# TensorSpeech/TensorFlowASR

Measured on AMD Instinct MI355X. Metric: audio-hours/sec (train step) Conformer-M RNN-T, higher is better.
Workload: dtype bf16; 1 GPU; Conformer-M transducer full train step (fwd+RNN-T loss+bwd+Adam), LibriSpeech-shaped 16 kHz utterances, 32/GPU, padding=batch, SpecAugment on, dropout 0.1; global_batch=32, parallelism=dp1, params=32461288

## Files before the change

### include/tfasr_hip.h

```cpp
#ifndef TFASR_HIP_H_
#define TFASR_HIP_H_

#include <stddef.h>
#include <stdint.h>

#ifdef __cplusplus
extern "C" {
#endif

#define TFASR_ABI_VERSION 44

typedef enum {
  TFASR_STATUS_SUCCESS = 0,
  TFASR_STATUS_INVALID_VALUE = 1,
  TFASR_STATUS_EXECUTION_FAILED = 2,
  TFASR_STATUS_UNSUPPORTED = 3
} tfasr_status_t;

typedef enum { TFASR_F32 = 0, TFASR_BF16 = 1 } tfasr_dtype_t;

const char* tfasr_status_string(int status);
int tfasr_abi_version(void);
size_t tfasr_launch_count(void);

// ... 3 lines not shown
                    int blank, int dtype, float* costs, void* workspace, size_t workspace_bytes,
                    void* stream);
int tfasr_rnnt_loss_packed_coef(const int32_t* labels, const int32_t* label_len, const int32_t* logit_len, const float* grad_scale,
                                const long* cell_off, long total_cells, const float* lse_part, int lse_parts, const float* pick, int B, int T,
                                int U1, int V, int blank, float* costs, float* coef, void* workspace, size_t workspace_bytes, void* stream);
int tfasr_rnnt_row_labels(const int32_t* labels, const int32_t* label_len, const int32_t* logit_len, const long* cell_off,
                          long total_cells, int B, int T, int U1, int V, int32_t* row_label, void* stream);
int tfasr_rnnt_loss_packed_stats(const void* logits, void* grads, const int32_t* labels, const int32_t* label_len,
                                 const int32_t* logit_len, const float* grad_scale, const long* cell_off, long total_cells,
                                 const float* lse_part, int lse_parts, const float* pick, int B, int T, int U1, int V, int blank,
                                 int dtype, float* costs, void* workspace, size_t workspace_bytes, void* stream);
int tfasr_rnnt_loss_packed(const void* logits, void* grads, const int32_t* labels, const int32_t* label_len,
                           const int32_t* logit_len, const float* grad_scale, const long* cell_off, long total_cells, int B,
                           int T, int U1, int V, int blank, int dtype, float* costs, void* workspace,
                           size_t workspace_bytes, void* stream);

int tfasr_ctc_loss_workspace_size(int B, int T, int U, int V, size_t* bytes);
int tfasr_ctc_loss(const void* logits, void* grads, const int32_t* labels, const int32_t* label_len,
                   const int32_t* logit_len, const float* grad_scale, int B, int T, int U, int V, int blank, int dtype,
                   float* costs, void* workspace, size_t workspace_bytes, void* stream);
int tfasr_ctc_greedy_decode(const void* logits, const int32_t* logit_len, int32_t* workspace_argmax, int32_t* tokens,
                            int32_t* tokens_len, int B, int T, int V, int blank, int dtype, void* stream);
int tfasr_ctc_greedy_decode_detail(const void* logits, const int32_t* logit_len, int32_t* workspace, int32_t* tokens, int32_t* tokens_len,
                                   int32_t* starts, int32_t* ends, float* tok_logp, float* tok_entropy, float* score, int B, int T, int V,
                                   int blank, int dtype, void* stream);

typedef enum { TFASR_ACT_NONE = 0, TFASR_ACT_SWISH = 1, TFASR_ACT_TANH = 2, TFASR_ACT_SIGMOID = 3, TFASR_ACT_TANH_OUT = 4,
               TFASR_ACT_FACTOR = 5  } tfasr_act_t;

typedef struct {
// ... 487 lines not shown
```

### tensorflowasr_amd/csrc/align.hip

```cpp
#include "common.h"
#include "lattice_lp.h"
#include <algorithm>

namespace {

typedef unsigned long long u64;

inline size_t align256(size_t x) { return (x + 255) & ~(size_t)255; }

constexpr int kRnntMaxU1 = TFASR_ALIGN_MAX_U1;
constexpr int kCtcMaxU = TFASR_ALIGN_CTC_MAX_U;

inline int rnnt_wave_e(int U1) { return U1 <= 64 ? 1 : (U1 <= 128 ? 2 : (U1 <= 256 ? 4 : 0)); }
inline int rnnt_dec_nw(int U1) { const int e = rnnt_wave_e(U1); return e ? e : (U1 + 63) / 64; }
inline size_t rnnt_dec_bytes(int B, int T, int U1) { return align256((size_t)B * ((size_t)T + U1) * rnnt_dec_nw(U1) * sizeof(u64)); }
inline int ctc_dec_nw(int U) { return (2 * U + 1 + 63) / 64; }

template <int E>
__global__ __launch_bounds__(64) void rnnt_viterbi_wave_kernel(const float* __restrict__ blank_lp, const float* __restrict__ truth_lp,
                                                               const int32_t* __restrict__ label_len, const int32_t* __restrict__ logit_len,
                                                               const long* __restrict__ cell_off, int Tm, int U1m, u64* __restrict__ dec,
                                                               long dec_stride, float* __restrict__ score) {
  const int b = blockIdx.x, lane = threadIdx.x;
  const int Tl = min(logit_len[b], Tm), Ul = max(min(label_len[b], U1m - 1), 0);
// ... 263 lines not shown
  if (!labels || !label_len || !logit_len || !score || !workspace || (U1 > 1 && (!frames || !label_lp))) return TFASR_STATUS_INVALID_VALUE;
  if (V <= 1 || blank < 0 || blank >= V) return TFASR_STATUS_INVALID_VALUE;
  const int st = rnnt_shape_status(B, T, U1);
  if (st != TFASR_STATUS_SUCCESS) return st;
  if (blank != 0) return TFASR_STATUS_UNSUPPORTED;
  const long nrows = cell_off ? total_cells : (long)B * T * U1;
  if (nrows <= 0 || nrows > (long)B * T * U1) return TFASR_STATUS_INVALID_VALUE;
  const size_t seg = align256((size_t)nrows * sizeof(float));
  if (workspace_bytes < 3 * seg + rnnt_dec_bytes(B, T, U1)) return TFASR_STATUS_INVALID_VALUE;
  hipStream_t stream = (hipStream_t)stream_;
  char* ws = (char*)workspace;
  float* lse = (float*)ws;
  float* bl = (float*)(ws + seg);
  float* tr = (float*)(ws + 2 * seg);
  const int lp = tfasr_detail::rnnt_lattice_logprobs(logits, labels, label_len, logit_len, cell_off, nrows, B, T, U1, V, dtype, lse_part, lse_parts,
                                                     pick, lse, bl, tr, stream);
  if (lp != TFASR_STATUS_SUCCESS) return lp;
  return rnnt_walk(bl, tr, label_len, logit_len, cell_off, B, T, U1, frames, label_lp, score, (u64*)(ws + 3 * seg), stream);
}

}

extern "C" int tfasr_rnnt_align_workspace_size(int B, int T, int U1, int V, size_t* bytes) {
  if (!bytes || V <= 0) return TFASR_STATUS_INVALID_VALUE;
  const int st = rnnt_shape_status(B, T, U1);
  if (st != TFASR_STATUS_SUCCESS) return st;
  *bytes = 3 * align256((size_t)B * T * U1 * sizeof(float)) + rnnt_dec_bytes(B, T, U1);
  return TFASR_STATUS_SUCCESS;
}

extern "C" int tfasr_rnnt_align_lattice(const float* blank_lp, const float* truth_lp, const int32_t* label_len, const int32_t* logit_len,
// ... 72 lines not shown
```

### tensorflowasr_amd/csrc/elementwise.hip

```cpp
#include "common.h"
#include <stdlib.h>
#include <algorithm>

namespace {

inline int flat_grid(long n, int per = 256) { return (int)std::max<long>(1, std::min<long>((n + per - 1) / per, 256L * 16)); }

template <typename S, typename D>
__global__ __launch_bounds__(256) void cast_kernel(const S* __restrict__ src, D* __restrict__ dst, long n) {
  const long n8 = n / 8;
  for (long i = (long)blockIdx.x * blockDim.x + threadIdx.x; i < n8; i += (long)gridDim.x * blockDim.x) {
    float v[8];
    ld8(src + i * 8, v);
    st8(dst + i * 8, v);
  }
  for (long i = n8 * 8 + (long)blockIdx.x * blockDim.x + threadIdx.x; i < n; i += (long)gridDim.x * blockDim.x)
    Num<D>::st(dst + i, Num<S>::ld(src + i));
}

template <typename T>
__global__ __launch_bounds__(256) void dropout_kernel(const T* x, T* y, long n, float p, uint64_t seed) {
  const long n8 = n / 8;
  const float inv = 1.f / (1.f - p);
  for (long i = (long)blockIdx.x * blockDim.x + threadIdx.x; i < n8; i += (long)gridDim.x * blockDim.x) {
// ... 522 lines not shown
    const float r = sqrtf(-2.0f * __logf(u1));
    float sn, cs;
    __sincosf(6.283185307179586f * u2, &sn, &cs);
    x[i] += stddev * r * ((i & 1) ? sn : cs);
  }
}

__global__ __launch_bounds__(256) void sumsq_kernel(const float* __restrict__ p, long n, float* __restrict__ out) {
  __shared__ float red[16];
  float a = 0.f;
  for (long i = (long)blockIdx.x * blockDim.x + threadIdx.x; i < n; i += (long)gridDim.x * blockDim.x) a += p[i] * p[i];
  a = block_sum(a, red);
  if (threadIdx.x == 0) atomicAdd(out, a);
}

template <typename T>
__global__ __launch_bounds__(256) void specaug_kernel(T* __restrict__ x, const int32_t* __restrict__ fmask,
                                                      const int32_t* __restrict__ tmask, int nf, int nt, int B, int Tn,
                                                      int F, float mval) {
  const long n = (long)B * Tn * F;
  for (long i = (long)blockIdx.x * blockDim.x + threadIdx.x; i < n; i += (long)gridDim.x * blockDim.x) {
    const int f = (int)(i % F);
    const int t = (int)((i / F) % Tn);
    const int b = (int)(i / ((long)F * Tn));
    bool hit = false;
    for (int k = 0; k < nf; ++k) {
      const int f0 = fmask[(b * nf + k) * 2], fw = fmask[(b * nf + k) * 2 + 1];
      hit |= (f >= f0 && f < f0 + fw);
    }
    for (int k = 0; k < nt; ++k) {
      const int t0 = tmask[(b * nt + k) * 2], tw = tmask[(b * nt + k) * 2 + 1];
      hit |= (t >= t0 && t < t0 + tw);
    }
    if (hit) Num<T>::st(x + i, mval);
  }
}

}

#define DISPATCH_T(dtype, CALL_F32, CALL_BF16) \
  do { if ((dtype) == TFASR_F32) { CALL_F32; } else if ((dtype) == TFASR_BF16) { CALL_BF16; } else return TFASR_STATUS_INVALID_VALUE; } while (0)

extern "C" int tfasr_cast(const void* src, void* dst, long n, int src_dtype, int dst_dtype, void* stream_) {
  if (!src || !dst || n <= 0) return TFASR_STATUS_INVALID_VALUE;
  hipStream_t s = (hipStream_t)stream_;
  const int grid = flat_grid(n / 8 + 1);
  if (src_dtype == TFASR_F32 && dst_dtype == TFASR_BF16)
    TFASR_KLAUNCH((cast_kernel<float, bf16_t>), dim3(grid), dim3(256), 0, s, (const float*)src, (bf16_t*)dst, n);
  else if (src_dtype == TFASR_BF16 && dst_dtype == TFASR_F32)
// ... 313 lines not shown
  TFASR_CHECK_LAUNCH();
  return TFASR_STATUS_SUCCESS;
}

extern "C" int tfasr_sumsq(const float* p, long n, float* out, void* stream_) {
  if (!p || !out || n <= 0) return TFASR_STATUS_INVALID_VALUE;
  TFASR_KLAUNCH(sumsq_kernel, dim3(flat_grid(n)), dim3(256), 0, (hipStream_t)stream_, p, n, out);
  TFASR_CHECK_LAUNCH();
  return TFASR_STATUS_SUCCESS;
}

extern "C" int tfasr_specaugment(void* x, const int32_t* fmask, const int32_t* tmask, int nf, int nt, int B, int T,
                                 int F, float mask_value, int dtype, void* stream_) {
  if (!x || B <= 0 || T <= 0 || F <= 0 || (nf > 0 && !fmask) || (nt > 0 && !tmask)) return TFASR_STATUS_INVALID_VALUE;
  hipStream_t s = (hipStream_t)stream_;
  const int grid = flat_grid((long)B * T * F);
  DISPATCH_T(dtype,
             TFASR_KLAUNCH(specaug_kernel<float>, dim3(grid), dim3(256), 0, s, (float*)x, fmask, tmask, nf, nt, B, T, F, mask_value),
             TFASR_KLAUNCH(specaug_kernel<bf16_t>, dim3(grid), dim3(256), 0, s, (bf16_t*)x, fmask, tmask, nf, nt, B, T, F, mask_value));
  TFASR_CHECK_LAUNCH();
  return TFASR_STATUS_SUCCESS;
}

namespace {
template <typename T>
__global__ __launch_bounds__(256) void add_pe_kernel(const T* __restrict__ x, const float* __restrict__ pe, const int32_t* __restrict__ lengths,
                                                     T* __restrict__ y, int B, int Tn, int d) {
  const int d8 = d / 8;
  const long n8 = (long)B * Tn * d8;
  for (long i = (long)blockIdx.x * blockDim.x + threadIdx.x; i < n8; i += (long)gridDim.x * blockDim.x) {
    const int c = (int)(i % d8) * 8;
    const long row = i / d8;
    const int t = (int)(row % Tn), b = (int)(row / Tn);
    float v[8];
// ... 23 lines not shown
```

### tensorflowasr_amd/csrc/lattice_lp.h

```cpp
#pragma once
#include "common.h"

namespace tfasr_detail {

__attribute__((visibility("hidden"))) int rnnt_lattice_logprobs(const void* logits, const int32_t* labels, const int32_t* label_len,
                                                                const int32_t* logit_len, const long* cell_off, long nrows, int B, int T, int U1,
                                                                int V, int dtype, const float* lse_part, int lse_parts, const float* pick,
                                                                float* lse, float* blank_lp, float* truth_lp, hipStream_t stream);

__attribute__((visibility("hidden"))) int ctc_row_lse(const void* logits, float* lse, long rows, int V, int dtype, hipStream_t stream);

}
```

### tensorflowasr_amd/csrc/rnnt_loss.hip

```cpp
#include "common.h"
#include "lattice_lp.h"
#include <algorithm>
#include <stdlib.h>

namespace {

struct RowStat { float m, s; };

__device__ __forceinline__ void online_add(RowStat& st, float x) {
  if (x > st.m) { st.s = st.s * __expf(st.m - x) + 1.f; st.m = x; }
  else          { st.s += __expf(x - st.m); }
}
__device__ __forceinline__ void online_merge(RowStat& a, float m2, float s2) {
  const float m = fmaxf(a.m, m2);
  if (m == -INFINITY) { a.m = m; a.s = 0.f; return; }
  a.s = a.s * __expf(a.m - m) + s2 * __expf(m2 - m);
  a.m = m;
}

struct Cell { int b, t, u, Tl, Ul; bool valid; };
__device__ __forceinline__ Cell locate(long r, const long* __restrict__ cell_off, int B, int Tm, int U1,
                                       const int32_t* __restrict__ label_len, const int32_t* __restrict__ logit_len) {
  Cell c;
  if (cell_off) {
    int lo = 0, hi = B;
    while (hi - lo > 1) { const int mid = (lo + hi) >> 1; if (cell_off[mid] <= r) lo = mid; else hi = mid; }
    c.b = lo;
    c.Tl = min(logit_len[lo], Tm); c.Ul = min(label_len[lo], U1 - 1);
    const long q = r - cell_off[lo];
    c.t = (int)(q / (c.Ul + 1)); c.u = (int)(q % (c.Ul + 1));
    c.valid = true;
  } else {
    c.u = (int)(r % U1); c.t = (int)((r / U1) % Tm); c.b = (int)(r / ((long)U1 * Tm));
    c.Tl = min(logit_len[c.b], Tm); c.Ul = min(label_len[c.b], U1 - 1);
    c.valid = (c.t < c.Tl && c.u <= c.Ul);
  }
  return c;
}

template <typename T>
__global__ __launch_bounds__(256) void rnnt_logprobs_kernel(
    const T* __restrict__ logits, const int32_t* __restrict__ labels, const int32_t* __restrict__ label_len,
    const int32_t* __restrict__ logit_len, const long* __restrict__ cell_off, long nrows, int B, int Tm, int U1, int V,
    float* __restrict__ lse, float* __restrict__ blank_lp, float* __restrict__ truth_lp) {
  const int lane = threadIdx.x & 63;
  const long wave0 = (long)blockIdx.x * (blockDim.x >> 6) + (threadIdx.x >> 6);
  const long nwaves = (long)gridDim.x * (blockDim.x >> 6);
  const bool vec_ok = (V % 8 == 0);
  for (long r = wave0; r < nrows; r += nwaves) {
    const Cell cl = locate(r, cell_off, B, Tm, U1, label_len, logit_len);
    const int u = cl.u, b = cl.b;
    if (!cl.valid) continue;
    const T* row = logits + r * V;
    RowStat st{-INFINITY, 0.f};
    int lab = -1;
    if (u < U1 - 1) lab = min(max(labels[(long)b * (U1 - 1) + u], 0), V - 1);
    float x_blank = 0.f, x_truth = 0.f;
    bool from_regs = false;
    if (vec_ok && V <= 2 * 64 * 8) {
// ... 37 lines not shown
          ld8(row + v0, x);
#pragma unroll
          for (int i = 0; i < 8; ++i) online_add(st, x[i]);
        }
      } else {
        for (int v = lane; v < V; v += 64) online_add(st, Num<T>::ld(row + v));
      }
#pragma unroll
      for (int o = 32; o > 0; o >>= 1) {
        const float m2 = __shfl_xor(st.m, o, 64), s2 = __shfl_xor(st.s, o, 64);
        online_merge(st, m2, s2);
      }
    }
    if (lane == 0) {
      const float l = st.m + logf(st.s);
      lse[r] = l;
      blank_lp[r] = (from_regs ? x_blank : Num<T>::ld(row)) - l;
      float tr = -INFINITY;
      if (lab >= 0) tr = (from_regs ? x_truth : Num<T>::ld(row + lab)) - l;
      truth_lp[r] = tr;
    }
  }
}

__global__ __launch_bounds__(256) void rnnt_row_labels_kernel(const int32_t* __restrict__ labels, const int32_t* __restrict__ label_len,
                                                              const int32_t* __restrict__ logit_len, const long* __restrict__ cell_off,
                                                              long nrows, int B, int Tm, int U1, int V, int32_t* __restrict__ row_label) {
  for (long r = (long)blockIdx.x * blockDim.x + threadIdx.x; r < nrows; r += (long)gridDim.x * blockDim.x) {
    const Cell cl = locate(r, cell_off, B, Tm, U1, label_len, logit_len);
    int lab = -1;
    if (cl.valid && cl.u < cl.Ul) lab = min(max(labels[(long)cl.b * (U1 - 1) + cl.u], 0), V - 1);
    row_label[r] = lab;
  }
}

__global__ __launch_bounds__(256) void rnnt_stats_finalize_kernel(const float2* __restrict__ part, int nparts, const float* __restrict__ pick,
                                                                  const int32_t* __restrict__ label_len, const int32_t* __restrict__ logit_len,
                                                                  const long* __restrict__ cell_off, long nrows, int B, int Tm, int U1,
                                                                  float* __restrict__ lse, float* __restrict__ blank_lp, float* __restrict__ truth_lp) {
  if (nparts == 16) {
    const int li = threadIdx.x & 15;
    const long g0 = ((long)blockIdx.x * blockDim.x + threadIdx.x) >> 4, gs = ((long)gridDim.x * blockDim.x) >> 4;
    const long nr16 = (nrows + gs - 1) / gs * gs;
    for (long r = g0; r < nr16; r += gs) {
      const bool in = r < nrows;
      const float2 v = in ? part[r * 16 + li] : make_float2(-INFINITY, 0.f);
      const float mx = row16_max(v.x);
      const float sm = row16_sum(v.y > 0.f ? v.y * __expf(v.x - mx) : 0.f);
      if (in && li == 0) {
        const Cell cl = locate(r, cell_off, B, Tm, U1, label_len, logit_len);
        if (cl.valid) {
          const float l = mx + logf(sm);
          const float2 pk = *reinterpret_cast<const float2*>(pick + 2 * r);
          lse[r] = l;
          blank_lp[r] = pk.x - l;
          truth_lp[r] = (cl.u < cl.Ul) ? pk.y - l : -INFINITY;
        }
      }
    }
    return;
  }
  for (long r = (long)blockIdx.x * blockDim.x + threadIdx.x; r < nrows; r += (long)gridDim.x * blockDim.x) {
    const Cell cl = locate(r, cell_off, B, Tm, U1, label_len, logit_len);
    if (!cl.valid) continue;
    RowStat st{-INFINITY, 0.f};
    for (int c = 0; c < nparts; ++c) {
      const float2 v = part[r * nparts + c];
      online_merge(st, v.x, v.y);
    }
    const float l = st.m + logf(st.s);
    lse[r] = l;
    blank_lp[r] = pick[2 * r] - l;
    truth_lp[r] = (cl.u < cl.Ul) ? pick[2 * r + 1] - l : -INFINITY;
  }
}

__device__ __forceinline__ void lds_barrier() { asm volatile("s_waitcnt lgkmcnt(0)\n\ts_barrier" ::: "memory"); }

__global__ __launch_bounds__(1024) void rnnt_lattice_kernel(const float* __restrict__ blank_lp, const float* __restrict__ truth_lp,
                                    const int32_t* __restrict__ label_len, const int32_t* __restrict__ logit_len,
                                    const long* __restrict__ cell_off, int Tm, int U1m, float* __restrict__ alpha,
                                    float* __restrict__ beta, float* __restrict__ costs) {
  extern __shared__ float sh[];
  const int b = blockIdx.x;
  const int u = threadIdx.x;
  const int nthr = blockDim.x;
  const int Tl = min(logit_len[b], Tm), Ul = min(label_len[b], U1m - 1);
  const int U1 = cell_off ? Ul + 1 : U1m;
// ... 85 lines not shown
        lds_barrier();
      }
    }
  }
}

template <bool FAST>
__device__ __forceinline__ float lae_(float a, float b) {
  if constexpr (!FAST) return logaddexpf_(a, b);
  const float m = fmaxf(a, b);
  if (m == -INFINITY) return -INFINITY;
  const float e = __builtin_amdgcn_exp2f(-fabsf(a - b) * 1.44269504088896340736f);
  return m + __builtin_amdgcn_logf(1.0f + e) * 0.69314718055994530942f;
}

template <int E, bool FAST>
__global__ __launch_bounds__(64) void rnnt_lattice_wave_kernel(const float* __restrict__ blank_lp, const float* __restrict__ truth_lp,
                                                               const int32_t* __restrict__ label_len, const int32_t* __restrict__ logit_len,
                                                               const long* __restrict__ cell_off, int Tm, int U1m, float* __restrict__ alpha,
                                                               float* __restrict__ beta, float* __restrict__ costs) {
  const int b = blockIdx.x, lane = threadIdx.x;
  const int Tl = min(logit_len[b], Tm), Ul = min(label_len[b], U1m - 1);
  const int U1 = cell_off ? Ul + 1 : U1m;
  const long base = cell_off ? cell_off[b] : (long)b * Tm * U1m;
  const float* bl = blank_lp + base;
  const float* tr = truth_lp + base;
  if (Tl <= 0) { if (lane == 0 && blockIdx.y == 1) costs[b] = 0.f; return; }
  const int ndiag = Tl + Ul;
  constexpr int PF = E == 1 ? 32 : (E == 2 ? 16 : 8);
  float rb[PF][E], rt[PF][E];
  int ue[E], uc[E];
  bool ucol[E];
#pragma unroll
  for (int e = 0; e < E; ++e) { ue[e] = lane * E + e; uc[e] = min(ue[e], Ul); ucol[e] = ue[e] <= Ul; }
  float self[E];
#pragma unroll
  for (int e = 0; e < E; ++e) self[e] = -INFINITY;
  if (blockIdx.y == 0) {
    float* al = alpha + base;
    auto fetch = [&](int n, int e, float& fb, float& ft) {
      const int tc = min(max(n - ue[e], 0), Tl - 1);
      fb = bl[max(tc - 1, 0) * U1 + uc[e]];
      ft = tr[tc * U1 + max(uc[e] - 1, 0)];
    };
#pragma unroll
    for (int j = 0; j < PF; ++j)
#pragma unroll
      for (int e = 0; e < E; ++e) fetch(j, e, rb[j][e], rt[j][e]);
    for (int n0 = 0; n0 < ndiag; n0 += PF) {
#pragma unroll
      for (int j = 0; j < PF; ++j) {
        const int n = n0 + j;
        float left[E];
        left[0] = __int_as_float(__builtin_amdgcn_update_dpp(__float_as_int(-INFINITY), __float_as_int(self[E - 1]), 0x138 , 0xf, 0xf, false));
#pragma unroll
        for (int e = 1; e < E; ++e) left[e] = self[e - 1];
#pragma unroll
        for (int e = 0; e < E; ++e) {
          const int t = n - ue[e];
          const bool act = ucol[e] && t >= 0 && t < Tl;
          const float pb = rb[j][e], pt = rt[j][e];
          fetch(n + PF, e, rb[j][e], rt[j][e]);
          if (act) {
            float a;
            if (t == 0 && ue[e] == 0) a = 0.f;
            else {
              const float xb = (t > 0) ? self[e] + pb : -INFINITY;
              const float xt = (ue[e] > 0) ? left[e] + pt : -INFINITY;
              a = lae_<FAST>(xb, xt);
            }
            al[t * U1 + ue[e]] = a;
            self[e] = a;
          }
        }
      }
    }
  } else {
    float* be = beta + base;
    auto fetch = [&](int it, int e, float& fb, float& ft) {
      const int tc = min(max((ndiag - 1 - it) - ue[e], 0), Tl - 1);
      fb = bl[tc * U1 + uc[e]];
      ft = tr[tc * U1 + uc[e]];
    };
#pragma unroll
    for (int j = 0; j < PF; ++j)
#pragma unroll
      for (int e = 0; e < E; ++e) fetch(j, e, rb[j][e], rt[j][e]);
    for (int i0 = 0; i0 < ndiag; i0 += PF) {
#pragma unroll
      for (int j = 0; j < PF; ++j) {
        const int it = i0 + j;
        const int n = ndiag - 1 - it;
        float right[E];
        right[E - 1] = __int_as_float(__builtin_amdgcn_update_dpp(__float_as_int(-INFINITY), __float_as_int(self[0]), 0x130 , 0xf, 0xf, false));
#pragma unroll
        for (int e = 0; e + 1 < E; ++e) right[e] = self[e + 1];
#pragma unroll
        for (int e = 0; e < E; ++e) {
          const int t = n - ue[e];
          const bool act = ucol[e] && t >= 0 && t < Tl;
          const float pb = rb[j][e], pt = rt[j][e];
          fetch(it + PF, e, rb[j][e], rt[j][e]);
          if (act) {
            float v;
            if (t == Tl - 1 && ue[e] == Ul) v = pb;
            else {
              const float xb = (t + 1 < Tl) ? self[e] + pb : -INFINITY;
              const float xt = (ue[e] < Ul) ? right[e] + pt : -INFINITY;
              v = lae_<FAST>(xb, xt);
            }
            be[t * U1 + ue[e]] = v;
            self[e] = v;
            if (t == 0 && ue[e] == 0) costs[b] = -v;
          }
        }
      }
    }
  }
}

template <typename T>
__global__ __launch_bounds__(256) void rnnt_grad_kernel(
    const T* logits, T* grads, const int32_t* __restrict__ labels,
    const int32_t* __restrict__ label_len, const int32_t* __restrict__ logit_len,
    const float* __restrict__ grad_scale, const long* __restrict__ cell_off, long nrows, int B, int Tm, int U1, int V,
    const float* __restrict__ lse, const float* __restrict__ blank_lp, const float* __restrict__ truth_lp,
    const float* __restrict__ alpha, const float* __restrict__ beta) {
  const int lane = threadIdx.x & 63;
  const long wave0 = (long)blockIdx.x * (blockDim.x >> 6) + (threadIdx.x >> 6);
  const long nwaves = (long)gridDim.x * (blockDim.x >> 6);
  const bool vec_ok = (V % 8 == 0);
  for (long r = wave0; r < nrows; r += nwaves) {
    const Cell cl = locate(r, cell_off, B, Tm, U1, label_len, logit_len);
    const int u = cl.u, t = cl.t, b = cl.b, Tl = cl.Tl, Ul = cl.Ul;
    const int ustride = cell_off ? Ul + 1 : U1;
    const T* row = logits + r * V;
    T* out = grads + r * V;
    if (!cl.valid) {
      if (vec_ok) {
        const float z[8] = {0, 0, 0, 0, 0, 0, 0, 0};
        for (int v0 = lane * 8; v0 < V; v0 += 64 * 8) st8(out + v0, z);
      } else {
        for (int v = lane; v < V; v += 64) Num<T>::st(out + v, 0.f);
      }
      continue;
    }
    const long lb = cell_off ? cell_off[b] : (long)b * Tm * U1;
    const float b00 = beta[lb];
    const float a = alpha[r];
    float gb = 0.f, gt = 0.f;
    if (t < Tl - 1) gb = -__expf(a + beta[r + ustride] + blank_lp[r] - b00);
    else if (u == Ul) gb = -1.f;
    int lab = -1;
    if (u < Ul) {
      gt = -__expf(a + beta[r + 1] + truth_lp[r] - b00);
      lab = min(max(labels[(long)b * (U1 - 1) + u], 0), V - 1);
    }
    const float sc = grad_scale ? grad_scale[b] : 1.f;
    const float l = lse[r];
    const float ssum = gb + gt;
    if (vec_ok) {
      const float l2 = l * 1.4426950408889634f, k1 = -ssum * sc, gbs = gb * sc, gts = gt * sc;
      for (int v0 = lane * 8; v0 < V; v0 += 64 * 8) {
        float x[8];
        ld8(row + v0, x);
#pragma unroll
        for (int i = 0; i < 8; ++i) x[i] = __builtin_amdgcn_exp2f(x[i] * 1.4426950408889634f - l2) * k1;
        if (v0 == 0) x[0] += gbs;
        if (lab >= 0 && (lab >> 3) == (v0 >> 3)) {
          const int q = lab & 7;
// ... 5 lines not shown
    } else {
      for (int v = lane; v < V; v += 64) {
        float g = -__expf(Num<T>::ld(row + v) - l) * ssum;
        if (v == 0) g += gb;
        if (v == lab) g += gt;
        Num<T>::st(out + v, g * sc);
      }
    }
  }
}

__global__ __launch_bounds__(256) void rnnt_coef_kernel(
    const int32_t* __restrict__ label_len, const int32_t* __restrict__ logit_len, const float* __restrict__ grad_scale,
    const long* __restrict__ cell_off, long nrows, int B, int Tm, int U1, const float* __restrict__ lse, const float* __restrict__ blank_lp,
    const float* __restrict__ truth_lp, const float* __restrict__ alpha, const float* __restrict__ beta, float4* __restrict__ coef,
    const int32_t* __restrict__ labels = nullptr, int V = 0, int32_t* __restrict__ rlab = nullptr) {
  for (long r = (long)blockIdx.x * blockDim.x + threadIdx.x; r < nrows; r += (long)gridDim.x * blockDim.x) {
    const Cell cl = locate(r, cell_off, B, Tm, U1, label_len, logit_len);
    float4 c = make_float4(3.0e38f, 0.f, 0.f, 0.f);
    if (rlab) rlab[r] = (cl.valid && cl.u < cl.Ul) ? min(max(labels[(long)cl.b * (U1 - 1) + cl.u], 0), V - 1) : -1;
    if (cl.valid) {
      const int u = cl.u, t = cl.t, b = cl.b, Tl = cl.Tl, Ul = cl.Ul;
      const int ustride = cell_off ? Ul + 1 : U1;
      const long lb = cell_off ? cell_off[b] : (long)b * Tm * U1;
      const float b00 = beta[lb], a = alpha[r];
      float gb = 0.f, gt = 0.f;
      if (t < Tl - 1) gb = -__expf(a + beta[r + ustride] + blank_lp[r] - b00);
      else if (u == Ul) gb = -1.f;
      if (u < Ul) gt = -__expf(a + beta[r + 1] + truth_lp[r] - b00);
      const float sc = grad_scale ? grad_scale[b] : 1.f;
      c = make_float4(lse[r] * 1.4426950408889634f, -(gb + gt) * sc, gb * sc, gt * sc);
    }
    coef[r] = c;
  }
}

template <typename T>
__global__ __launch_bounds__(256) void rnnt_grad_apply_kernel(const T* __restrict__ logits, T* __restrict__ grads, const float4* __restrict__ coef,
                                                              const int32_t* __restrict__ rlab, long nrows, int V) {
  const int lane = threadIdx.x & 63;
  const long wave0 = (long)blockIdx.x * (blockDim.x >> 6) + (threadIdx.x >> 6);
  const long nwaves = (long)gridDim.x * (blockDim.x >> 6);
  constexpr int U = 2, MAXP = 2;
  for (long r0 = wave0; r0 < nrows; r0 += U * nwaves) {
// ... 38 lines not shown
}

inline size_t align256(size_t x) { return (x + 255) & ~(size_t)255; }

}

extern "C" int tfasr_rnnt_loss_workspace_size(int B, int T, int U1, int V, size_t* bytes) {
  if (!bytes || B <= 0 || T <= 0 || U1 <= 0 || V <= 0) return TFASR_STATUS_INVALID_VALUE;
  const size_t n = (size_t)B * T * U1;
  *bytes = 10 * align256(n * sizeof(float));
  return TFASR_STATUS_SUCCESS;
}

int tfasr_detail::rnnt_lattice_logprobs(const void* logits, const int32_t* labels, const int32_t* label_len, const int32_t* logit_len,
                                        const long* cell_off, long nrows, int B, int T, int U1, int V, int dtype, const float* lse_part,
                                        int lse_parts, const float* pick, float* lse, float* blank_lp, float* truth_lp, hipStream_t stream) {
  const int wpb = 4;
  const int grid = (int)std::min<long>((nrows + wpb - 1) / wpb, 256L * 32);
  if (lse_part) {
    const int fg = (int)std::min<long>(((lse_parts == 16 ? nrows * 16 : nrows) + 255) / 256, 256L * 16);
    TFASR_KLAUNCH(rnnt_stats_finalize_kernel, dim3(fg), dim3(256), 0, stream, (const float2*)lse_part, lse_parts, pick, label_len, logit_len,
                       cell_off, nrows, B, T, U1, lse, blank_lp, truth_lp);
  } else if (dtype == TFASR_F32)
    TFASR_KLAUNCH(rnnt_logprobs_kernel<float>, dim3(grid), dim3(256), 0, stream, (const float*)logits, labels,
                       label_len, logit_len, cell_off, nrows, B, T, U1, V, lse, blank_lp, truth_lp);
  else if (dtype == TFASR_BF16)
    TFASR_KLAUNCH(rnnt_logprobs_kernel<bf16_t>, dim3(grid), dim3(256), 0, stream, (const bf16_t*)logits, labels,
                       label_len, logit_len, cell_off, nrows, B, T, U1, V, lse, blank_lp, truth_lp);
  else
    return TFASR_STATUS_INVALID_VALUE;
  TFASR_CHECK_LAUNCH();
  return TFASR_STATUS_SUCCESS;
}

static int rnnt_impl(const void* logits, void* grads, const int32_t* labels, const int32_t* label_len,
                     const int32_t* logit_len, const float* grad_scale, const long* cell_off, long nrows, int B, int T, int U1,
                     int V, int blank, int dtype, float* costs, void* workspace, size_t workspace_bytes, void* stream_,
                     const float* lse_part = nullptr, int lse_parts = 0, const float* pick = nullptr, float* coef = nullptr) {
  if ((!logits && !(lse_part && coef && !grads)) || !labels || !label_len || !logit_len || !costs || !workspace) return TFASR_STATUS_INVALID_VALUE;
  if (blank != 0) return TFASR_STATUS_UNSUPPORTED;
  if (B <= 0 || T <= 0 || U1 <= 0 || V <= 1 || U1 > 1024 || nrows <= 0) return TFASR_STATUS_INVALID_VALUE;
  const size_t n = (size_t)nrows;
  const size_t seg = align256(n * sizeof(float));
  if (workspace_bytes < 5 * seg) return TFASR_STATUS_INVALID_VALUE;
  hipStream_t stream = (hipStream_t)stream_;
  char* ws = (char*)workspace;
  float* lse = (float*)(ws);
  float* blank_lp = (float*)(ws + seg);
  float* truth_lp = (float*)(ws + 2 * seg);
  float* alpha = (float*)(ws + 3 * seg);
  float* beta = (float*)(ws + 4 * seg);
  const int wpb = 4;
  int grid = (int)std::min<long>((nrows + wpb - 1) / wpb, 256L * 32);
  const int lp_status = tfasr_detail::rnnt_lattice_logprobs(logits, labels, label_len, logit_len, cell_off, nrows, B, T, U1, V, dtype, lse_part,
                                                            lse_parts, pick, lse, blank_lp, truth_lp, stream);
  if (lp_status != TFASR_STATUS_SUCCESS) return lp_status;
  const int nthr = ((U1 + 63) / 64) * 64;
  static const bool wave_off = false;
  static const bool fast = !(false);
#define TFASR_LW(E) do { if (fast) TFASR_KLAUNCH((rnnt_lattice_wave_kernel<E, true>), dim3(B, 2), dim3(64), 0, stream, blank_lp, truth_lp, label_len, logit_len, cell_off, T, U1, alpha, beta, costs); \
                         else TFASR_KLAUNCH((rnnt_lattice_wave_kernel<E, false>), dim3(B, 2), dim3(64), 0, stream, blank_lp, truth_lp, label_len, logit_len, cell_off, T, U1, alpha, beta, costs); } while (0)
  if (!wave_off && U1 <= 64) TFASR_LW(1);
  else if (!wave_off && U1 <= 128) TFASR_LW(2);
  else if (!wave_off && U1 <= 256) TFASR_LW(4);
  else
    TFASR_KLAUNCH(rnnt_lattice_kernel, dim3(B, 2), dim3(nthr), 2 * nthr * sizeof(float), stream, blank_lp,
                       truth_lp, label_len, logit_len, cell_off, T, U1, alpha, beta, costs);
  TFASR_CHECK_LAUNCH();
  static const bool stream_off = false;
  const bool streamed = grads && !stream_off && (V % 8) == 0 && V <= 1024 && workspace_bytes >= 10 * seg && (dtype == TFASR_F32 || dtype == TFASR_BF16);
  float4* cbuf = coef ? (float4*)coef : (float4*)(ws + 5 * seg);
  int32_t* rlab = (int32_t*)(ws + 9 * seg);
  if (coef || streamed) {
    const int cg = (int)std::min<long>((nrows + 255) / 256, 256L * 8);
    TFASR_KLAUNCH(rnnt_coef_kernel, dim3(cg), dim3(256), 0, stream, label_len, logit_len, grad_scale, cell_off, nrows, B, T, U1, lse, blank_lp,
                       truth_lp, alpha, beta, cbuf, streamed ? labels : (const int32_t*)nullptr, V, streamed ? rlab : (int32_t*)nullptr);
    TFASR_CHECK_LAUNCH();
  }
  if (streamed) {
    const int ag = (int)std::min<long>((nrows + 7) / 8, 256L * 16);
    if (dtype == TFASR_F32)
      TFASR_KLAUNCH(rnnt_grad_apply_kernel<float>, dim3(ag), dim3(256), 0, stream, (const float*)logits, (float*)grads, cbuf, rlab, nrows, V);
    else
      TFASR_KLAUNCH(rnnt_grad_apply_kernel<bf16_t>, dim3(ag), dim3(256), 0, stream, (const bf16_t*)logits, (bf16_t*)grads, cbuf, rlab, nrows, V);
    TFASR_CHECK_LAUNCH();
    return TFASR_STATUS_SUCCESS;
  }
  if (grads) {
    if (dtype == TFASR_F32)
      TFASR_KLAUNCH(rnnt_grad_kernel<float>, dim3(grid), dim3(256), 0, stream, (const float*)logits,
                         (float*)grads, labels, label_len, logit_len, grad_scale, cell_off, nrows, B, T, U1, V, lse, blank_lp,
                         truth_lp, alpha, beta);
    else
      TFASR_KLAUNCH(rnnt_grad_kernel<bf16_t>, dim3(grid), dim3(256), 0, stream, (const bf16_t*)logits,
                         (bf16_t*)grads, labels, label_len, logit_len, grad_scale, cell_off, nrows, B, T, U1, V, lse, blank_lp,
                         truth_lp, alpha, beta);
    TFASR_CHECK_LAUNCH();
  }
  return TFASR_STATUS_SUCCESS;
}

extern "C" int tfasr_rnnt_loss(const void* logits, void* grads, const int32_t* labels, const int32_t* label_len,
                               const int32_t* logit_len, const float* grad_scale, int B, int T, int U1, int V,
                               int blank, int dtype, float* costs, void* workspace, size_t workspace_bytes,
                               void* stream_) {
  return rnnt_impl(logits, grads, labels, label_len, logit_len, grad_scale, nullptr, (long)B * T * U1, B, T, U1, V, blank, dtype,
                   costs, workspace, workspace_bytes, stream_);
}

extern "C" int tfasr_rnnt_loss_packed(const void* logits, void* grads, const int32_t* labels, const int32_t* label_len,
                                      const int32_t* logit_len, const float* grad_scale, const long* cell_off, long total_cells,
// ... 35 lines not shown
```

### tensorflowasr_amd/kernels.py

```python
import ctypes
import os

import torch

from . import _lib
from ._lib import ACT_FACTOR, ACT_NONE, ACT_SIGMOID, ACT_SWISH, ACT_TANH, ACT_TANH_OUT, TFASR_BF16, TFASR_F32, GemmArgs, check

_WS_CACHE = {}
_SPLITK_WS = False


def _dt(t):
    if t.dtype == torch.float32:
        return TFASR_F32
    if t.dtype == torch.bfloat16:
        return TFASR_BF16
    raise TypeError(f"unsupported activation dtype {t.dtype}")


def _p(t):
    if t is None:
        return None
    if not t.is_cuda:
        raise _lib.TfasrError("tensorflowasr_amd ops need HIP device tensors (no CPU fallback on the product path)")
# ... 20 lines not shown


def workspace(nbytes, device, tag="ws"):
    key = (str(device), tag)
    buf = _WS_CACHE.get(key)
    if buf is None or buf.numel() < nbytes:
        buf = torch.empty(max(int(nbytes), 256), dtype=torch.uint8, device=device)
        _WS_CACHE[key] = buf
    return buf


def rnnt_loss_workspace_size(B, T, U1, V):
    n = ctypes.c_size_t(0)
    check(_lib.load().tfasr_rnnt_loss_workspace_size(B, T, U1, V, ctypes.byref(n)), "rnnt_loss_workspace_size")
    return n.value


def rnnt_loss_fwd_bwd(logits, labels, label_len, logit_len, grad_scale=None, grads=None, want_grads=True, blank=0):
    assert logits.dim() == 4 and logits.is_contiguous()
    B, T, U1, V = logits.shape
    assert labels.shape == (B, U1 - 1) and labels.dtype == torch.int32 and labels.is_contiguous()
    assert label_len.dtype == torch.int32 and logit_len.dtype == torch.int32
    costs = torch.empty(B, dtype=torch.float32, device=logits.device)
    if want_grads and grads is None:
        grads = torch.empty_like(logits)
    nbytes = rnnt_loss_workspace_size(B, T, U1, V)
    ws = workspace(nbytes, logits.device, "rnnt")
    check(
        _lib.load().tfasr_rnnt_loss(
            _p(logits), _p(grads) if want_grads else None, _p(labels), _p(label_len), _p(logit_len),
# ... 1845 lines not shown
```

Before: 4.746 audio-hours/sec.

## Skew RNN-T lattice storage along diagonals and rewrite SpecAugment as row-range fills

The RNN-T lattice log-probs, alpha and beta are now stored in a skewed layout where row index is (t+u) mod Tl. Each anti-diagonal step of the wavefront kernel then reads and writes one contiguous row instead of strided cells. The wavefront body is made branch-free, and the grad and coef kernels remap their indices to match. SpecAugment is also rewritten separately: masked time ranges get vectorized fills and frequency bands get per-row strided writes, replacing a per-element check over every mask. The cost is more complex indexing (modulo arithmetic) and a new global layout switch that defaults to skewed.

```diff
diff --git a/include/tfasr_hip.h b/include/tfasr_hip.h
--- a/include/tfasr_hip.h
+++ b/include/tfasr_hip.h
@@ -41,6 +41,9 @@
                            const int32_t* logit_len, const float* grad_scale, const long* cell_off, long total_cells, int B,
                            int T, int U1, int V, int blank, int dtype, float* costs, void* workspace,
                            size_t workspace_bytes, void* stream);
+#define TFASR_LATTICE_ROW_MAJOR 0
+#define TFASR_LATTICE_SKEWED 1
+int tfasr_rnnt_set_lattice_layout(int layout);
 
 int tfasr_ctc_loss_workspace_size(int B, int T, int U, int V, size_t* bytes);
 int tfasr_ctc_loss(const void* logits, void* grads, const int32_t* labels, const int32_t* label_len,
diff --git a/tensorflowasr_amd/csrc/align.hip b/tensorflowasr_amd/csrc/align.hip
--- a/tensorflowasr_amd/csrc/align.hip
+++ b/tensorflowasr_amd/csrc/align.hip
@@ -301,7 +301,7 @@
   float* bl = (float*)(ws + seg);
   float* tr = (float*)(ws + 2 * seg);
   const int lp = tfasr_detail::rnnt_lattice_logprobs(logits, labels, label_len, logit_len, cell_off, nrows, B, T, U1, V, dtype, lse_part, lse_parts,
-                                                     pick, lse, bl, tr, stream);
+                                                     pick, lse, bl, tr, TFASR_LATTICE_ROW_MAJOR, stream);
   if (lp != TFASR_STATUS_SUCCESS) return lp;
   return rnnt_walk(bl, tr, label_len, logit_len, cell_off, B, T, U1, frames, label_lp, score, (u64*)(ws + 3 * seg), stream);
 }
diff --git a/tensorflowasr_amd/csrc/elementwise.hip b/tensorflowasr_amd/csrc/elementwise.hip
--- a/tensorflowasr_amd/csrc/elementwise.hip
+++ b/tensorflowasr_amd/csrc/elementwise.hip
@@ -560,25 +560,58 @@
   if (threadIdx.x == 0) atomicAdd(out, a);
 }
 
+constexpr int SPECAUG_ROWS = 64;
 template <typename T>
 __global__ __launch_bounds__(256) void specaug_kernel(T* __restrict__ x, const int32_t* __restrict__ fmask,
                                                       const int32_t* __restrict__ tmask, int nf, int nt, int B, int Tn,
                                                       int F, float mval) {
-  const long n = (long)B * Tn * F;
-  for (long i = (long)blockIdx.x * blockDim.x + threadIdx.x; i < n; i += (long)gridDim.x * blockDim.x) {
-    const int f = (int)(i % F);
-    const int t = (int)((i / F) % Tn);
-    const int b = (int)(i / ((long)F * Tn));
-    bool hit = false;
+  extern __shared__ int32_t sm[];
+  int32_t* fr = sm;
+  int32_t* trg = sm + 2 * nf;
+  const int b = blockIdx.y;
+  const int r0 = blockIdx.x * SPECAUG_ROWS, r1 = min(r0 + SPECAUG_ROWS, Tn);
+  for (int k = threadIdx.x; k < nf; k += blockDim.x) {
+    const long f0 = fmask[((long)b * nf + k) * 2], fw = fmask[((long)b * nf + k) * 2 + 1];
+    fr[2 * k] = (int)max(f0, 0L);
+    fr[2 * k + 1] = (int)min(f0 + fw, (long)F);
+  }
+  for (int k = threadIdx.x; k < nt; k += blockDim.x) {
+    const long t0 = tmask[((long)b * nt + k) * 2], tw = tmask[((long)b * nt + k) * 2 + 1];
+    trg[2 * k] = (int)max(t0, (long)r0);
+    trg[2 * k + 1] = (int)min(t0 + tw, (long)r1);
+  }
+  __syncthreads();
+  T one;
+  Num<T>::st(&one, mval);
+  T* xb = x + (long)b * Tn * F;
+  constexpr int PER = 16 / (int)sizeof(T);
+  uint32_t w;
+  if constexpr (sizeof(T) == 2) w = (uint32_t)one * 0x10001u; else w = __float_as_uint(one);
+  const uint4 pat = make_uint4(w, w, w, w);
+  for (int k = 0; k < nt; ++k) {
+    const int ta = trg[2 * k], tb = trg[2 * k + 1];
+    if (tb <= ta) continue;
+    T* p = xb + (long)ta * F;
+    const long n = (long)(tb - ta) * F;
+    const long head = min(n, (long)(((16 - (int)((uintptr_t)p & 15)) & 15) / (int)sizeof(T)));
+    const long nv = (n - head) / PER;
+    if (threadIdx.x < head) p[threadIdx.x] = one;
+    uint4* pv = reinterpret_cast<uint4*>(p + head);
+    for (long i = threadIdx.x; i < nv; i += blockDim.x) pv[i] = pat;
+    const long done = head + nv * PER;
+    if (done + threadIdx.x < n) p[done + threadIdx.x] = one;
+  }
+  if (nf <= 0) return;
+  const int lane = threadIdx.x & 31;
+  for (int t = r0 + (threadIdx.x >> 5); t < r1; t += 8) {
+    bool masked = false;
+    for (int k = 0; k < nt; ++k) masked |= (t >= trg[2 * k] && t < trg[2 * k + 1]);
+    if (masked) continue;
+    T* row = xb + (long)t * F;
     for (int k = 0; k < nf; ++k) {
-      const int f0 = fmask[(b * nf + k) * 2], fw = fmask[(b * nf + k) * 2 + 1];
-      hit |= (f >= f0 && f < f0 + fw);
+      const int fb = fr[2 * k + 1];
+      for (int f = fr[2 * k] + lane; f < fb; f += 32) row[f] = one;
     }
-    for (int k = 0; k < nt; ++k) {
-      const int t0 = tmask[(b * nt + k) * 2], tw = tmask[(b * nt + k) * 2 + 1];
-      hit |= (t >= t0 && t < t0 + tw);
-    }
-    if (hit) Num<T>::st(x + i, mval);
   }
 }
 
@@ -922,10 +955,15 @@
                                  int F, float mask_value, int dtype, void* stream_) {
   if (!x || B <= 0 || T <= 0 || F <= 0 || (nf > 0 && !fmask) || (nt > 0 && !tmask)) return TFASR_STATUS_INVALID_VALUE;
   hipStream_t s = (hipStream_t)stream_;
-  const int grid = flat_grid((long)B * T * F);
-  DISPATCH_T(dtype,
-             TFASR_KLAUNCH(specaug_kernel<float>, dim3(grid), dim3(256), 0, s, (float*)x, fmask, tmask, nf, nt, B, T, F, mask_value),
-             TFASR_KLAUNCH(specaug_kernel<bf16_t>, dim3(grid), dim3(256), 0, s, (bf16_t*)x, fmask, tmask, nf, nt, B, T, F, mask_value));
+  nf = std::max(nf, 0); nt = std::max(nt, 0);
+  if (dtype != TFASR_F32 && dtype != TFASR_BF16) return TFASR_STATUS_INVALID_VALUE;
+  if (nf + nt == 0) return TFASR_STATUS_SUCCESS;
+  if (nf + nt > 4096 || B > 65535) return TFASR_STATUS_UNSUPPORTED;
+  const dim3 grid((T + SPECAUG_ROWS - 1) / SPECAUG_ROWS, B);
+  const size_t lds = (size_t)(nf + nt) * 2 * sizeof(int32_t);
+  DISPATCH_T(dtype,
+             TFASR_KLAUNCH(specaug_kernel<float>, grid, dim3(256), lds, s, (float*)x, fmask, tmask, nf, nt, B, T, F, mask_value),
+             TFASR_KLAUNCH(specaug_kernel<bf16_t>, grid, dim3(256), lds, s, (bf16_t*)x, fmask, tmask, nf, nt, B, T, F, mask_value));
   TFASR_CHECK_LAUNCH();
   return TFASR_STATUS_SUCCESS;
 }
diff --git a/tensorflowasr_amd/csrc/lattice_lp.h b/tensorflowasr_amd/csrc/lattice_lp.h
--- a/tensorflowasr_amd/csrc/lattice_lp.h
+++ b/tensorflowasr_amd/csrc/lattice_lp.h
@@ -6,7 +6,7 @@
 __attribute__((visibility("hidden"))) int rnnt_lattice_logprobs(const void* logits, const int32_t* labels, const int32_t* label_len,
                                                                 const int32_t* logit_len, const long* cell_off, long nrows, int B, int T, int U1,
                                                                 int V, int dtype, const float* lse_part, int lse_parts, const float* pick,
-                                                                float* lse, float* blank_lp, float* truth_lp, hipStream_t stream);
+                                                                float* lse, float* blank_lp, float* truth_lp, int layout, hipStream_t stream);
 
 __attribute__((visibility("hidden"))) int ctc_row_lse(const void* logits, float* lse, long rows, int V, int dtype, hipStream_t stream);
 
diff --git a/tensorflowasr_amd/csrc/rnnt_loss.hip b/tensorflowasr_amd/csrc/rnnt_loss.hip
--- a/tensorflowasr_amd/csrc/rnnt_loss.hip
+++ b/tensorflowasr_amd/csrc/rnnt_loss.hip
@@ -38,11 +38,18 @@
   return c;
 }
 
+__device__ __forceinline__ long lattice_slot(long lb, int U1s, int Tl, int t, int u, bool skew) {
+  return lb + (long)(skew ? (t + u) % Tl : t) * U1s + u;
+}
+__device__ __forceinline__ long lattice_base(const Cell& c, const long* __restrict__ cell_off, int Tm, int U1) {
+  return cell_off ? cell_off[c.b] : (long)c.b * Tm * U1;
+}
+
 template <typename T>
 __global__ __launch_bounds__(256) void rnnt_logprobs_kernel(
     const T* __restrict__ logits, const int32_t* __restrict__ labels, const int32_t* __restrict__ label_len,
     const int32_t* __restrict__ logit_len, const long* __restrict__ cell_off, long nrows, int B, int Tm, int U1, int V,
-    float* __restrict__ lse, float* __restrict__ blank_lp, float* __restrict__ truth_lp) {
+    float* __restrict__ lse, float* __restrict__ blank_lp, float* __restrict__ truth_lp, bool skew) {
   const int lane = threadIdx.x & 63;
   const long wave0 = (long)blockIdx.x * (blockDim.x >> 6) + (threadIdx.x >> 6);
   const long nwaves = (long)gridDim.x * (blockDim.x >> 6);
@@ -110,11 +117,12 @@
     }
     if (lane == 0) {
       const float l = st.m + logf(st.s);
+      const long q = skew ? lattice_slot(lattice_base(cl, cell_off, Tm, U1), cell_off ? cl.Ul + 1 : U1, cl.Tl, cl.t, u, true) : r;
       lse[r] = l;
-      blank_lp[r] = (from_regs ? x_blank : Num<T>::ld(row)) - l;
+      blank_lp[q] = (from_regs ? x_blank : Num<T>::ld(row)) - l;
       float tr = -INFINITY;
       if (lab >= 0) tr = (from_regs ? x_truth : Num<T>::ld(row + lab)) - l;
-      truth_lp[r] = tr;
+      truth_lp[q] = tr;
     }
   }
 }
@@ -133,7 +141,8 @@
 __global__ __launch_bounds__(256) void rnnt_stats_finalize_kernel(const float2* __restrict__ part, int nparts, const float* __restrict__ pick,
                                                                   const int32_t* __restrict__ label_len, const int32_t* __restrict__ logit_len,
                                                                   const long* __restrict__ cell_off, long nrows, int B, int Tm, int U1,
-                                                                  float* __restrict__ lse, float* __restrict__ blank_lp, float* __restrict__ truth_lp) {
+                                                                  float* __restrict__ lse, float* __restrict__ blank_lp, float* __restrict__ truth_lp,
+                                                                  bool skew) {
   if (nparts == 16) {
     const int li = threadIdx.x & 15;
     const long g0 = ((long)blockIdx.x * blockDim.x + threadIdx.x) >> 4, gs = ((long)gridDim.x * blockDim.x) >> 4;
@@ -148,9 +157,10 @@
         if (cl.valid) {
           const float l = mx + logf(sm);
           const float2 pk = *reinterpret_cast<const float2*>(pick + 2 * r);
+          const long q = skew ? lattice_slot(lattice_base(cl, cell_off, Tm, U1), cell_off ? cl.Ul + 1 : U1, cl.Tl, cl.t, cl.u, true) : r;
           lse[r] = l;
-          blank_lp[r] = pk.x - l;
-          truth_lp[r] = (cl.u < cl.Ul) ? pk.y - l : -INFINITY;
+          blank_lp[q] = pk.x - l;
+          truth_lp[q] = (cl.u < cl.Ul) ? pk.y - l : -INFINITY;
         }
       }
     }
@@ -165,9 +175,10 @@
       online_merge(st, v.x, v.y);
     }
     const float l = st.m + logf(st.s);
+    const long q = skew ? lattice_slot(lattice_base(cl, cell_off, Tm, U1), cell_off ? cl.Ul + 1 : U1, cl.Tl, cl.t, cl.u, true) : r;
     lse[r] = l;
-    blank_lp[r] = pick[2 * r] - l;
-    truth_lp[r] = (cl.u < cl.Ul) ? pick[2 * r + 1] - l : -INFINITY;
+    blank_lp[q] = pick[2 * r] - l;
+    truth_lp[q] = (cl.u < cl.Ul) ? pick[2 * r + 1] - l : -INFINITY;
   }
 }
 
@@ -283,7 +294,7 @@
   return m + __builtin_amdgcn_logf(1.0f + e) * 0.69314718055994530942f;
 }
 
-template <int E, bool FAST>
+template <int E, bool FAST, bool SKEW>
 __global__ __launch_bounds__(64) void rnnt_lattice_wave_kernel(const float* __restrict__ blank_lp, const float* __restrict__ truth_lp,
                                                                const int32_t* __restrict__ label_len, const int32_t* __restrict__ logit_len,
                                                                const long* __restrict__ cell_off, int Tm, int U1m, float* __restrict__ alpha,
@@ -307,15 +318,25 @@
   for (int e = 0; e < E; ++e) self[e] = -INFINITY;
   if (blockIdx.y == 0) {
     float* al = alpha + base;
+    const int wrap = Tl * U1;
+    int frow = wrap - U1, wrow = 0;
+    auto next_row = [&](int& o) { o += U1; if (o == wrap) o = 0; };
     auto fetch = [&](int n, int e, float& fb, float& ft) {
-      const int tc = min(max(n - ue[e], 0), Tl - 1);
-      fb = bl[max(tc - 1, 0) * U1 + uc[e]];
-      ft = tr[tc * U1 + max(uc[e] - 1, 0)];
+      if constexpr (SKEW) {
+        fb = bl[frow + uc[e]];
+        ft = tr[frow + max(uc[e] - 1, 0)];
+      } else {
+        const int tc = min(max(n - ue[e], 0), Tl - 1);
+        fb = bl[max(tc - 1, 0) * U1 + uc[e]];
+        ft = tr[tc * U1 + max(uc[e] - 1, 0)];
+      }
     };
 #pragma unroll
-    for (int j = 0; j < PF; ++j)
+    for (int j = 0; j < PF; ++j) {
 #pragma unroll
       for (int e = 0; e < E; ++e) fetch(j, e, rb[j][e], rt[j][e]);
+      next_row(frow);
+    }
     for (int n0 = 0; n0 < ndiag; n0 += PF) {
 #pragma unroll
       for (int j = 0; j < PF; ++j) {
@@ -330,31 +351,38 @@
           const bool act = ucol[e] && t >= 0 && t < Tl;
           const float pb = rb[j][e], pt = rt[j][e];
           fetch(n + PF, e, rb[j][e], rt[j][e]);
-          if (act) {
-            float a;
-            if (t == 0 && ue[e] == 0) a = 0.f;
-            else {
-              const float xb = (t > 0) ? self[e] + pb : -INFINITY;
-              const float xt = (ue[e] > 0) ? left[e] + pt : -INFINITY;
-              a = lae_<FAST>(xb, xt);
-            }
-            al[t * U1 + ue[e]] = a;
-            self[e] = a;
-          }
-        }
+          const float xb = (t > 0) ? self[e] + pb : -INFINITY;
+          const float xt = (ue[e] > 0) ? left[e] + pt : -INFINITY;
+          float a = lae_<FAST>(xb, xt);
+          if (t == 0 && ue[e] == 0) a = 0.f;
+          if (act) al[SKEW ? wrow + ue[e] : t * U1 + ue[e]] = a;
+          self[e] = act ? a : self[e];
+        }
+        next_row(frow);
+        next_row(wrow);
       }
     }
   } else {
     float* be = beta + base;
+    const int wrap = Tl * U1;
+    int frow = ((ndiag - 1) % Tl) * U1, wrow = frow;
+    auto prev_row = [&](int& o) { if (o == 0) o = wrap; o -= U1; };
     auto fetch = [&](int it, int e, float& fb, float& ft) {
-      const int tc = min(max((ndiag - 1 - it) - ue[e], 0), Tl - 1);
-      fb = bl[tc * U1 + uc[e]];
-      ft = tr[tc * U1 + uc[e]];
+      if constexpr (SKEW) {
+        fb = bl[frow + uc[e]];
+        ft = tr[frow + uc[e]];
+      } else {
+        const int tc = min(max((ndiag - 1 - it) - ue[e], 0), Tl - 1);
+        fb = bl[tc * U1 + uc[e]];
+        ft = tr[tc * U1 + uc[e]];
+      }
     };
 #pragma unroll
-    for (int j = 0; j < PF; ++j)
+    for (int j = 0; j < PF; ++j) {
 #pragma unroll
       for (int e = 0; e < E; ++e) fetch(j, e, rb[j][e], rt[j][e]);
+      prev_row(frow);
+    }
     for (int i0 = 0; i0 < ndiag; i0 += PF) {
 #pragma unroll
       for (int j = 0; j < PF; ++j) {
@@ -370,19 +398,18 @@
           const bool act = ucol[e] && t >= 0 && t < Tl;
           const float pb = rb[j][e], pt = rt[j][e];
           fetch(it + PF, e, rb[j][e], rt[j][e]);
+          const float xb = (t + 1 < Tl) ? self[e] + pb : -INFINITY;
+          const float xt = (ue[e] < Ul) ? right[e] + pt : -INFINITY;
+          float v = lae_<FAST>(xb, xt);
+          if (t == Tl - 1 && ue[e] == Ul) v = pb;
           if (act) {
-            float v;
-            if (t == Tl - 1 && ue[e] == Ul) v = pb;
-            else {
-              const float xb = (t + 1 < Tl) ? self[e] + pb : -INFINITY;
-              const float xt = (ue[e] < Ul) ? right[e] + pt : -INFINITY;
-              v = lae_<FAST>(xb, xt);
-            }
-            be[t * U1 + ue[e]] = v;
-            self[e] = v;
+            be[SKEW ? wrow + ue[e] : t * U1 + ue[e]] = v;
             if (t == 0 && ue[e] == 0) costs[b] = -v;
           }
-        }
+          self[e] = act ? v : self[e];
+        }
+        prev_row(frow);
+        prev_row(wrow);
       }
     }
   }
@@ -394,7 +421,7 @@
     const int32_t* __restrict__ label_len, const int32_t* __restrict__ logit_len,
     const float* __restrict__ grad_scale, const long* __restrict__ cell_off, long nrows, int B, int Tm, int U1, int V,
     const float* __restrict__ lse, const float* __restrict__ blank_lp, const float* __restrict__ truth_lp,
-    const float* __restrict__ alpha, const float* __restrict__ beta) {
+    const float* __restrict__ alpha, const float* __restrict__ beta, bool skew) {
   const int lane = threadIdx.x & 63;
   const long wave0 = (long)blockIdx.x * (blockDim.x >> 6) + (threadIdx.x >> 6);
   const long nwaves = (long)gridDim.x * (blockDim.x >> 6);
@@ -416,13 +443,16 @@
     }
     const long lb = cell_off ? cell_off[b] : (long)b * Tm * U1;
     const float b00 = beta[lb];
-    const float a = alpha[r];
+    const long q = skew ? lattice_slot(lb, ustride, Tl, t, u, true) : r;
+    const long qd = skew ? lattice_slot(lb, ustride, Tl, t + 1, u, true) : r + ustride;
+    const long qr = skew ? qd + 1 : r + 1;
+    const float a = alpha[q];
     float gb = 0.f, gt = 0.f;
-    if (t < Tl - 1) gb = -__expf(a + beta[r + ustride] + blank_lp[r] - b00);
+    if (t < Tl - 1) gb = -__expf(a + beta[qd] + blank_lp[q] - b00);
     else if (u == Ul) gb = -1.f;
     int lab = -1;
     if (u < Ul) {
-      gt = -__expf(a + beta[r + 1] + truth_lp[r] - b00);
+      gt = -__expf(a + beta[qr] + truth_lp[q] - b00);
       lab = min(max(labels[(long)b * (U1 - 1) + u], 0), V - 1);
     }
     const float sc = grad_scale ? grad_scale[b] : 1.f;
@@ -458,7 +488,7 @@
     const int32_t* __restrict__ label_len, const int32_t* __restrict__ logit_len, const float* __restrict__ grad_scale,
     const long* __restrict__ cell_off, long nrows, int B, int Tm, int U1, const float* __restrict__ lse, const float* __restrict__ blank_lp,
     const float* __restrict__ truth_lp, const float* __restrict__ alpha, const float* __restrict__ beta, float4* __restrict__ coef,
-    const int32_t* __restrict__ labels = nullptr, int V = 0, int32_t* __restrict__ rlab = nullptr) {
+    const int32_t* __restrict__ labels, int V, int32_t* __restrict__ rlab, bool skew) {
   for (long r = (long)blockIdx.x * blockDim.x + threadIdx.x; r < nrows; r += (long)gridDim.x * blockDim.x) {
     const Cell cl = locate(r, cell_off, B, Tm, U1, label_len, logit_len);
     float4 c = make_float4(3.0e38f, 0.f, 0.f, 0.f);
@@ -467,11 +497,14 @@
       const int u = cl.u, t = cl.t, b = cl.b, Tl = cl.Tl, Ul = cl.Ul;
       const int ustride = cell_off ? Ul + 1 : U1;
       const long lb = cell_off ? cell_off[b] : (long)b * Tm * U1;
-      const float b00 = beta[lb], a = alpha[r];
+      const long q = skew ? lattice_slot(lb, ustride, Tl, t, u, true) : r;
+      const long qd = skew ? lattice_slot(lb, ustride, Tl, t + 1, u, true) : r + ustride;
+      const long qr = skew ? qd + 1 : r + 1;
+      const float b00 = beta[lb], a = alpha[q];
       float gb = 0.f, gt = 0.f;
-      if (t < Tl - 1) gb = -__expf(a + beta[r + ustride] + blank_lp[r] - b00);
+      if (t < Tl - 1) gb = -__expf(a + beta[qd] + blank_lp[q] - b00);
       else if (u == Ul) gb = -1.f;
-      if (u < Ul) gt = -__expf(a + beta[r + 1] + truth_lp[r] - b00);
+      if (u < Ul) gt = -__expf(a + beta[qr] + truth_lp[q] - b00);
       const float sc = grad_scale ? grad_scale[b] : 1.f;
       c = make_float4(lse[r] * 1.4426950408889634f, -(gb + gt) * sc, gb * sc, gt * sc);
     }
@@ -540,23 +573,32 @@
 
 int tfasr_detail::rnnt_lattice_logprobs(const void* logits, const int32_t* labels, const int32_t* label_len, const int32_t* logit_len,
                                         const long* cell_off, long nrows, int B, int T, int U1, int V, int dtype, const float* lse_part,
-                                        int lse_parts, const float* pick, float* lse, float* blank_lp, float* truth_lp, hipStream_t stream) {
+                                        int lse_parts, const float* pick, float* lse, float* blank_lp, float* truth_lp, int layout,
+                                        hipStream_t stream) {
+  const bool skew = layout == TFASR_LATTICE_SKEWED;
   const int wpb = 4;
   const int grid = (int)std::min<long>((nrows + wpb - 1) / wpb, 256L * 32);
   if (lse_part) {
     const int fg = (int)std::min<long>(((lse_parts == 16 ? nrows * 16 : nrows) + 255) / 256, 256L * 16);
     TFASR_KLAUNCH(rnnt_stats_finalize_kernel, dim3(fg), dim3(256), 0, stream, (const float2*)lse_part, lse_parts, pick, label_len, logit_len,
-                       cell_off, nrows, B, T, U1, lse, blank_lp, truth_lp);
+                       cell_off, nrows, B, T, U1, lse, blank_lp, truth_lp, skew);
   } else if (dtype == TFASR_F32)
     TFASR_KLAUNCH(rnnt_logprobs_kernel<float>, dim3(grid), dim3(256), 0, stream, (const float*)logits, labels,
-                       label_len, logit_len, cell_off, nrows, B, T, U1, V, lse, blank_lp, truth_lp);
+                       label_len, logit_len, cell_off, nrows, B, T, U1, V, lse, blank_lp, truth_lp, skew);
   else if (dtype == TFASR_BF16)
     TFASR_KLAUNCH(rnnt_logprobs_kernel<bf16_t>, dim3(grid), dim3(256), 0, stream, (const bf16_t*)logits, labels,
-                       label_len, logit_len, cell_off, nrows, B, T, U1, V, lse, blank_lp, truth_lp);
+                       label_len, logit_len, cell_off, nrows, B, T, U1, V, lse, blank_lp, truth_lp, skew);
   else
     return TFASR_STATUS_INVALID_VALUE;
   TFASR_CHECK_LAUNCH();
   return TFASR_STATUS_SUCCESS;
+}
+
+static int g_lattice_layout = TFASR_LATTICE_SKEWED;
+extern "C" int tfasr_rnnt_set_lattice_layout(int layout) {
+  const int prev = g_lattice_layout;
+  if (layout == TFASR_LATTICE_ROW_MAJOR || layout == TFASR_LATTICE_SKEWED) g_lattice_layout = layout;
+  return prev;
 }
 
 static int rnnt_impl(const void* logits, void* grads, const int32_t* labels, const int32_t* label_len,
@@ -578,14 +620,17 @@
   float* beta = (float*)(ws + 4 * seg);
   const int wpb = 4;
   int grid = (int)std::min<long>((nrows + wpb - 1) / wpb, 256L * 32);
+  static const bool wave_off = false;
+  static const bool fast = !(false);
+  const bool skew = !wave_off && U1 <= 256 && g_lattice_layout == TFASR_LATTICE_SKEWED;
   const int lp_status = tfasr_detail::rnnt_lattice_logprobs(logits, labels, label_len, logit_len, cell_off, nrows, B, T, U1, V, dtype, lse_part,
-                                                            lse_parts, pick, lse, blank_lp, truth_lp, stream);
+                                                            lse_parts, pick, lse, blank_lp, truth_lp,
+                                                            skew ? TFASR_LATTICE_SKEWED : TFASR_LATTICE_ROW_MAJOR, stream);
   if (lp_status != TFASR_STATUS_SUCCESS) return lp_status;
   const int nthr = ((U1 + 63) / 64) * 64;
-  static const bool wave_off = false;
-  static const bool fast = !(false);
-#define TFASR_LW(E) do { if (fast) TFASR_KLAUNCH((rnnt_lattice_wave_kernel<E, true>), dim3(B, 2), dim3(64), 0, stream, blank_lp, truth_lp, label_len, logit_len, cell_off, T, U1, alpha, beta, costs); \
-                         else TFASR_KLAUNCH((rnnt_lattice_wave_kernel<E, false>), dim3(B, 2), dim3(64), 0, stream, blank_lp, truth_lp, label_len, logit_len, cell_off, T, U1, alpha, beta, costs); } while (0)
+#define TFASR_LW2(E, F, S) TFASR_KLAUNCH((rnnt_lattice_wave_kernel<E, F, S>), dim3(B, 2), dim3(64), 0, stream, blank_lp, truth_lp, label_len, logit_len, cell_off, T, U1, alpha, beta, costs)
+#define TFASR_LW(E) do { if (fast) { if (skew) TFASR_LW2(E, true, true); else TFASR_LW2(E, true, false); } \
+                         else { if (skew) TFASR_LW2(E, false, true); else TFASR_LW2(E, false, false); } } while (0)
   if (!wave_off && U1 <= 64) TFASR_LW(1);
   else if (!wave_off && U1 <= 128) TFASR_LW(2);
   else if (!wave_off && U1 <= 256) TFASR_LW(4);
@@ -600,7 +645,7 @@
   if (coef || streamed) {
     const int cg = (int)std::min<long>((nrows + 255) / 256, 256L * 8);
     TFASR_KLAUNCH(rnnt_coef_kernel, dim3(cg), dim3(256), 0, stream, label_len, logit_len, grad_scale, cell_off, nrows, B, T, U1, lse, blank_lp,
-                       truth_lp, alpha, beta, cbuf, streamed ? labels : (const int32_t*)nullptr, V, streamed ? rlab : (int32_t*)nullptr);
+                       truth_lp, alpha, beta, cbuf, streamed ? labels : (const int32_t*)nullptr, V, streamed ? rlab : (int32_t*)nullptr, skew);
     TFASR_CHECK_LAUNCH();
   }
   if (streamed) {
@@ -616,11 +661,11 @@
     if (dtype == TFASR_F32)
       TFASR_KLAUNCH(rnnt_grad_kernel<float>, dim3(grid), dim3(256), 0, stream, (const float*)logits,
                          (float*)grads, labels, label_len, logit_len, grad_scale, cell_off, nrows, B, T, U1, V, lse, blank_lp,
-                         truth_lp, alpha, beta);
+                         truth_lp, alpha, beta, skew);
     else
       TFASR_KLAUNCH(rnnt_grad_kernel<bf16_t>, dim3(grid), dim3(256), 0, stream, (const bf16_t*)logits,
                          (bf16_t*)grads, labels, label_len, logit_len, grad_scale, cell_off, nrows, B, T, U1, V, lse, blank_lp,
-                         truth_lp, alpha, beta);
+                         truth_lp, alpha, beta, skew);
     TFASR_CHECK_LAUNCH();
   }
   return TFASR_STATUS_SUCCESS;
diff --git a/tensorflowasr_amd/kernels.py b/tensorflowasr_amd/kernels.py
--- a/tensorflowasr_amd/kernels.py
+++ b/tensorflowasr_amd/kernels.py
@@ -58,6 +58,10 @@
     n = ctypes.c_size_t(0)
     check(_lib.load().tfasr_rnnt_loss_workspace_size(B, T, U1, V, ctypes.byref(n)), "rnnt_loss_workspace_size")
     return n.value
+
+
+def rnnt_set_lattice_layout(layout):
+    return int(_L().tfasr_rnnt_set_lattice_layout(int(layout)))
 
 
 def rnnt_loss_fwd_bwd(logits, labels, label_len, logit_len, grad_scale=None, grads=None, want_grads=True, blank=0):
```

Result: no change. 4.758 audio-hours/sec (median of 6 runs) (+0.3%).
